# zhide1983/audio_codec

Measured on AMD Instinct MI355X. Metric: Mframes/s encoded (48kHz/10ms/64kbps), higher is better.
Workload: dtype f32

## Files before the change

audio_codec_amd/csrc/lc3_enc_front4.inc:

```
#define F4_FR 4
#define F4_N 480
#define F4_CS 36
#define F4_ZS 544
struct __attribute__((aligned(16))) Front4Lds {
    float x[MEMCAP + F4_FR * F4_N + 4];
    float scr[364];
    int   pc[LC3D_PLAN_HEAD_WORDS];
    int   cc[14];
};
static_assert(MEMCAP % 4 == 0 && F4_FR * F4_ZS <= MEMCAP + F4_FR * F4_N, "front4 work buffers fit into the PCM area");

__device__ __forceinline__ void f4_dft240x4(float* x, const lc3d_plan* __restrict__ P, float norm, int lane)
{
    constexpr int N = F4_N;
    {
        const int f = lane >> 4, col = lane & 15;
        if (col < 15) {
            float* z = &x[F4_ZS * f + F4_CS * col];
            float v[32];
#pragma unroll
            for (int q = 0; q < 8; q++) { const float4 u = *(const float4*)&z[4 * q]; v[4 * q] = u.x; v[4 * q + 1] = u.y; v[4 * q + 2] = u.z; v[4 * q + 3] = u.w; }
            dft16(v);
#pragma unroll
            for (int q = 0; q < 8; q++) *(float4*)&z[4 * q] = make_float4(v[4 * q], v[4 * q + 1], v[4 * q + 2], v[4 * q + 3]);
        }
    }
    LSYNC();
    {
        const int f = lane >> 4, row = lane & 15;
        float v[30];
#pragma unroll
        for (int l = 0; l < 15; l++) { const float2 u = *(const float2*)&x[F4_ZS * f + F4_CS * l + 2 * row]; v[2 * l] = u.x; v[2 * l + 1] = u.y; }
        dft15(v);
        float o0[15], o1[15];
#pragma unroll
        for (int l = 0; l < 15; l++) {
            const unsigned tt = 15u * row + 16u * l, d = tt < tt - 240u ? tt : tt - 240u;
            const float2 tw = *(const float2*)&P->tw2[2 * d];
            const float ar = v[2 * l], ai = v[2 * l + 1];
            const float tr = ar * tw.x - ai * tw.y, ti = ai * tw.x + ar * tw.y;
            o0[l] = tr * norm; o1[l] = -ti * norm;
        }
        LSYNC();
        float* A = &x[N * f];
#pragma unroll
        for (int l = 0; l < 15; l++) {
            const unsigned tt = 15u * row + 16u * l, d = tt < tt - 240u ? tt : tt - 240u;
            A[2 * d] = o0[l]; A[N - 2 * d - 1] = o1[l];
        }
    }
    LSYNC();
}

#ifndef F4_WAVES
#define F4_WAVES 4
#endif
extern "C" __global__ void __launch_bounds__(WAVE) __attribute__((amdgpu_waves_per_eu(F4_WAVES, F4_WAVES)))
#ifdef LC3_PCM_FMT
lc3_enc_front4_kernel_fmt(
#else
lc3_enc_front4_kernel(
#endif
                      const lc3d_plan* __restrict__ P, const lc3d_chan* __restrict__ chans, const float* __restrict__ state, const void* __restrict__ pcm, int bitdepth,
                      int T, int tb, int nt , int ncs, float* __restrict__ spec, int srow, int RT, int r0, float* __restrict__ rec,
                      float* __restrict__ xnext, const float* __restrict__ xprev, int xprev_stride)
{
    __shared__ Front4Lds L;
    const int lane = threadIdx.x;
    const int runs = (nt + F4_FR - 1) / F4_FR;
    const int cs = blockIdx.x / runs, t0 = tb + (blockIdx.x % runs) * F4_FR, nf = imin(F4_FR, tb + nt - t0);
    if (cs >= ncs) return;
    if (lane < LC3D_PLAN_HEAD_WORDS) L.pc[lane] = ((const int*)P)[lane];
    if (lane < 14) L.cc[lane] = ((const int*)&chans[cs])[lane];
    LSYNC();
    constexpr int N = F4_N, h = N / 2;
    const int channels = PI(channels);
    const int strm = cs / channels, ch = cs - strm * channels;
#ifndef LC3_PCM_FMT
    const float sc = bitdepth == 24 ? 256.0f : 65536.0f;
#endif
#ifdef LC3_PCM_FMT
    {
        const int ps = lc3d_pcm_stride(bitdepth, channels);
        const size_t pf0 = lc3d_pcm_frame(bitdepth, channels, T, N, strm, t0, ch), pfst = lc3d_pcm_fstep(bitdepth, channels, N);
        const bool fastf = pcm_f32_wide(pcm, bitdepth, pf0, N) && ((pfst * 4) & 15) == 0;
        if (t0 == 0) { for (int i = lane; i < MEMCAP; i += WAVE) L.x[i] = xprev[(size_t)cs * xprev_stride + i]; }
        else {
            const size_t pidx = pf0 - pfst + (size_t)(N - MEMCAP) * ps;
            if (fastf) {
                const float4* p = (const float4*)((const float*)pcm + pidx);
                for (int j = lane; j < MEMCAP / 4; j += WAVE) *(float4*)&L.x[4 * j] = pcm_f32x4(p[j]);
            } else for (int j = lane; j < MEMCAP; j += WAVE) L.x[j] = pcm_in(pcm, bitdepth, pidx + (size_t)j * ps);
        }
        if (fastf) {
            for (int idx = lane; idx < 120 * nf; idx += WAVE) {
                const int f = idx / 120, j = idx - 120 * f;
                *(float4*)&L.x[MEMCAP + N * f + 4 * j] = pcm_f32x4(((const float4*)((const float*)pcm + pf0 + (size_t)f * pfst))[j]);
            }
        } else {
            for (int f = 0; f < nf; f++) {
                const size_t o = pf0 + (size_t)f * pfst;
                for (int i = lane; i < N; i += WAVE) L.x[MEMCAP + N * f + i] = pcm_in(pcm, bitdepth, o + (size_t)i * ps);
            }
        }
    }
#else
    {
        const size_t f0 = ((size_t)strm * T + t0) * channels + ch;
        const bool fast = bitdepth == 16 && (((size_t)pcm) & 15) == 0;
        if (t0 == 0) { for (int i = lane; i < MEMCAP; i += WAVE) L.x[i] = xprev[(size_t)cs * xprev_stride + i]; }
        else {
            const size_t pidx = (f0 - channels) * N + (N - MEMCAP);
            if (fast) {
                const uint2* p = (const uint2*)((const int16_t*)pcm + pidx);
                for (int j = lane; j < MEMCAP / 4; j += WAVE) {
                    const uint2 v = p[j];
                    *(float4*)&L.x[4 * j] = make_float4((float)(int16_t)(v.x & 0xffff), (float)(int16_t)(v.x >> 16), (float)(int16_t)(v.y & 0xffff), (float)(int16_t)(v.y >> 16));
                }
            } else for (int j = lane; j < MEMCAP; j += WAVE)
                L.x[j] = bitdepth == 16 ? (float)((const int16_t*)pcm)[pidx + j] : (float)((const int32_t*)pcm)[pidx + j] / sc;
        }
        if (fast) {
#pragma unroll
            for (int k = 0; k < 4; k++) {
                const int idx = lane + 64 * k, f = idx / 60, j = idx - 60 * f;
                if (idx < 240 && f < nf) {
#ifdef F4_NOLOAD
                    const uint4 v = make_uint4(idx * 77u, idx * 131u, idx * 17u, idx * 3u);
#else
                    const uint4 v = ((const uint4*)((const int16_t*)pcm + (f0 + (size_t)f * channels) * N))[j];
#endif
                    float* d = &L.x[MEMCAP + N * f + 8 * j];
                    *(float4*)&d[0] = make_float4((float)(int16_t)(v.x & 0xffff), (float)(int16_t)(v.x >> 16), (float)(int16_t)(v.y & 0xffff), (float)(int16_t)(v.y >> 16));
                    *(float4*)&d[4] = make_float4((float)(int16_t)(v.z & 0xffff), (float)(int16_t)(v.z >> 16), (float)(int16_t)(v.w & 0xffff), (float)(int16_t)(v.w >> 16));
                }
            }
        } else {
            for (int f = 0; f < nf; f++) {
                const size_t o = (f0 + (size_t)f * channels) * N;
                for (int i = lane; i < N; i += WAVE)
                    L.x[MEMCAP + N * f + i] = bitdepth == 16 ? (float)((const int16_t*)pcm)[o + i] : (float)((const int32_t*)pcm)[o + i] / sc;
            }
        }
    }
#endif
    LSYNC();
    if (t0 + nf == T) for (int i = lane; i < MEMCAP; i += WAVE) xnext[(size_t)cs * MEMCAP + i] = L.x[N * nf + i];
    float* r = rec + ((size_t)cs * RT + r0 + t0) * FR_WORDS;
    if (lane < nf) ((int*)r)[(size_t)lane * FR_WORDS + FR_ATTFLAG] = 0;
    if (CI(attack_handling) != 0) {
        const float* stp = state + (size_t)cs * LC3D_STATE_WORDS(MEMCAP);
        float am0 = 0, am1 = 0;
        for (int f = 0; f < nf; f++) {
            if (t0 + f == 0) { if (!CI(reset_attack)) { am0 = stp[LC3D_ST_SCAL(MEMCAP) + F_ATT_M0]; am1 = stp[LC3D_ST_SCAL(MEMCAP) + F_ATT_M1]; } }
            else if (f == 0) { const float* q = &L.x[MEMCAP]; am0 = (q[-6] + q[-5] + q[-4]); am1 = (q[-3] + q[-2] + q[-1]); }
            float n0, n1;
            const float e = attack_energies_at(PI(att_nblocks), 48000, &L.x[MEMCAP + N * f], L.scr, lane, am0, am1, n0, n1);
            float* rf = r + (size_t)f * FR_WORDS;
            if (lane < 4) rf[FR_ATT + lane] = lane < PI(att_nblocks) ? e : 0.0f;
            if (lane == 0) { rf[FR_ATTM] = n0; rf[FR_ATTM + 1] = n1; }
            am0 = n0; am1 = n1;
            LSYNC();
        }
    }
    const float* w = &lc3t_win_pool[PI(win_off)];
    const int lim = 2 * N - PI(la);
    float zr[4][F4_FR], zi[4][F4_FR];
    if (lane < 60) {
#pragma unroll
        for (int k = 0; k < 4; k++) {
            const int i = lane + 60 * k;
            const int m1 = k < 2 ? 2 * i : N - 1 - 2 * i, m2 = k < 2 ? h - 1 - 2 * i : 2 * i - h;
            const int j0 = 3 * h - m1 - 1, j1 = 3 * h + m1, j2 = m2, j3 = 2 * h - m2 - 1;
            const float w0 = w[j0], w1 = w[j1], w2 = w[j2], w3 = w[j3];
            const float2 tw = *(const float2*)&P->tw1[2 * i];
            const bool in1 = j1 < lim; const int j1c = in1 ? j1 : 0;
#pragma unroll
            for (int f = 0; f < F4_FR; f++) {
                const float* t = &L.x[N * f];
                const float a0 = t[j0] * w0;
                const float a1 = (in1 ? t[j1c] : 0.0f) * w1;
                const float a2 = t[j2] * w2;
                const float a3 = t[j3] * w3;
                const float F1 = -a0 - a1, F2 = a2 - a3;
                const float ar = k < 2 ? F1 : F2, ai = k < 2 ? F2 : F1;
                zr[k][f] = ar * tw.x - ai * tw.y;
                zi[k][f] = ai * tw.x + ar * tw.y;
            }
        }
    }
    LSYNC();
    if (lane < 60) {
#pragma unroll
        for (int k = 0; k < 4; k++) {
            const int i = lane + 60 * k;
            const int o = (i % 15) * F4_CS + 2 * (i & 15);
#pragma unroll
            for (int f = 0; f < F4_FR; f++) *(float2*)&L.x[F4_ZS * f + o] = make_float2(zr[k][f], zi[k][f]);
        }
    }
    LSYNC();
    f4_dft240x4(L.x, P, PF(dct4_norm), lane);
    {
        const int nq = PI(ylen);
        float* base = LC3D_ROW_BASE(spec, cs, r0 + t0, RT, srow);
        for (int idx = lane; idx < nq; idx += WAVE) {
            const int c = idx >> 4, f = (idx >> 2) & 3, q = idx & 3;
            if (f < nf) *(float4*)&base[((size_t)c * RT + f) * 16 + 4 * q] = *(const float4*)&L.x[N * f + 16 * c + 4 * q];
        }
    }
}
```

audio_codec_amd/csrc/lc3_enc_shapel.inc:

```
#ifndef LC3_BIG
struct __attribute__((aligned(16))) ShlLds {
    double l10[128 * 3];
    double ex2[64];
    unsigned bob[LC3D_MAX_N / 4];
    int   pc[LC3D_PLAN_HEAD_WORDS];
};

__device__ __attribute__((noinline)) void shl_lpc_weight(const float* a_in, const float* rc_in, float* outp, int maxOrder, float maxPG, float predGain)
{
    float sc[36], pa[9];
    pa[0] = 1;
    for (int j = 1; j <= maxOrder - 1; j++) pa[j] = -a_in[maxOrder - j];
    pa[maxOrder] = rc_in[maxOrder - 1];
    const float alpha = (float)((double)((maxPG - predGain)) * (0.85f - 1.0) / (double)(maxPG - 1.5f) + 1.0);
    for (int i = 0; i <= maxOrder; i++) sc[i] = pa[i] * m_powf(alpha, (float)i);
    int len = maxOrder + 1; const int len0 = len;
    float* pa_ = sc; float* out = sc + 9; float* t0 = sc + 18; float* bf = sc + 26;
    for (int i = 0; i < len - 1; i++) out[i] = 0;
    { float a0 = pa_[0]; for (int i = 0; i < len; i++) { pa_[i] = pa_[i] / a0; a0 = pa_[0]; } }
    out[len - 1] = pa_[len - 1];
    for (int k = len0 - 2; k >= 0; k--) {
        for (int i = 0; i < len - 1; i++) t0[i] = pa_[1 + i];
        int l = len - 1;
        const float knxt = t0[l - 1];
// ... 18 lines not shown
#define SHL_ATTR __attribute__((amdgpu_waves_per_eu(SHL_WAVES, SHL_WAVES), amdgpu_num_vgpr(SHL_VGPRS)))
#else
#define SHL_ATTR __attribute__((amdgpu_waves_per_eu(SHL_WAVES, SHL_WAVES)))
#endif
#ifdef LC3_ENC_VBW
#define SHL_KERNEL_NAME lc3_enc_shape_lane_kernel_vbw
#else
#define SHL_KERNEL_NAME lc3_enc_shape_lane_kernel
#endif
extern "C" __global__ void __launch_bounds__(WAVE) SHL_ATTR
SHL_KERNEL_NAME(const lc3d_plan* __restrict__ P, const lc3d_chan* __restrict__ chans, int RT , int r0 , int nt, int ncs,
                          float* __restrict__ rows , int srow, float* __restrict__ frec
#ifdef LC3_ENC_VBW
                          , const uint16_t* __restrict__ bwf
#endif
                          )
{
    __shared__ ShlLds L;
    const int lane = threadIdx.x;
    if (lane < LC3D_PLAN_HEAD_WORDS) L.pc[lane] = ((const int*)P)[lane];
    for (int i = lane; i < LC3D_MAX_N; i += WAVE) ((uint8_t*)L.bob)[i] = P->band_of_bin[i];
    for (int i = lane; i < 128 * 3; i += WAVE) L.l10[i] = lc3m_log10_tab[i];
    L.ex2[lane] = lc3m_exp2_tab[lane];
    LSYNC();
#if !defined(LC3_OCML_MATH) && !defined(SHL_GLOBAL_TABLES)
#define m_log10f(x_) lc3m_log10f((x_), L.l10)
#define m_pow2f(x_) lc3m_exp2f((x_), L.ex2)
#endif
    const long long cf = (long long)blockIdx.x * WAVE + lane;
    const bool valid = cf < (long long)ncs * nt;
    const int cs = valid ? (int)(cf / nt) : 0, t = valid ? r0 + (int)(cf % nt) : r0;
    float* xr = LC3D_ROW_BASE(rows, cs, t, RT, srow);
#define XP(k_) (&xr[LC3D_ROW_OFF((k_), RT)])
    float* rec = frec + ((size_t)cs * RT + t) * FR_WORDS;
    const lc3d_chan* __restrict__ C = &chans[cs];
    const int ylen = PI(ylen), N = PI(N), nb = PI(nbands), dms = PI(dms), hr = PI(hrmode);
    const int total_bits = C->total_bits, off = C->gg_off;
    float g[16];
#pragma unroll
    for (int i = 0; i < 16; i += 4) { const float4 v = *(const float4*)&rec[FR_SCFQ + i]; g[i] = v.x; g[i + 1] = v.y; g[i + 2] = v.z; g[i + 3] = v.w; }
    const int dnb = 64 - nb;
    int n4 = 0;
    if (dnb >= 32) { const float ratio = fabsf((float)(1.0 - 32.0 / (double)(float)nb)); n4 = (int)round((double)(ratio * (float)nb)); }
    auto v64 = [&](int i) -> float {
        float ga, gb; int r;
        if (i < 2) return g[0];
        if (i < 62) { const int n = (i - 2) >> 2; r = (i - 2) & 3; ga = g[n]; gb = g[n + 1]; }
        else { ga = g[15]; gb = g[15]; r = i - 62; const double dd = (double)(g[15] - g[14]); return r == 0 ? (float)((double)ga + dd / 8.0) : (float)((double)ga + 3.0 * dd / 8.0); }
        const double dd = (double)(gb - ga);
        if (r == 0) return (float)((double)ga + dd / 8.0);
        if (r == 1) return (float)((double)ga + 3.0 * dd / 8.0);
        if (r == 2) return (float)((double)ga + 5.0 * dd / 8.0);
        return (float)((double)ga + 7.0 * dd / 8.0);
    };
    auto band_gain = [&](int b) -> float {
        float v;
        if (dnb == 0) v = v64(b);
        else if (dnb < 32) { if (b < dnb) v = (float)((double)(v64(2 * b) + v64(2 * b + 1)) / 2.0); else v = v64(b + dnb); }
        else {
            if (b < n4) v = (float)((double)(v64(4 * b) + v64(4 * b + 1) + v64(4 * b + 2) + v64(4 * b + 3)) / 4.0);
            else { const int i = b - n4; v = (float)((double)(v64(4 * n4 + 2 * i) + v64(4 * n4 + 2 * i + 1)) / 2.0); }
        }
        return m_pow2f(-v);
    };
    int bw = ((const int*)rec)[FR_BW];
#ifdef LC3_ENC_VBW
// ... 5 lines not shown
    if (cut) bw = imin(bw, C->bw_index);
#endif
    const int bw_bin = lc3t_bw_bins[PI(bw_cls) * 6 + bw];
    int numfilters, start0, start1 = 0, stop0, stop1 = 0, obits_off = 8; float maxPG = 2;
    const int maxOrder = dms == 100 ? 8 : 4, nSub = dms == 100 ? 3 : 2;
    {
        int fs = PI(fs), Nn = N;
        numfilters = (fs >= 32000 && dms >= 50) ? 2 : 1;
        if ((double)Nn > 40 * ((double)(float)dms / 10.0)) { Nn = (int)(40 * ((double)(float)dms / 10.0)); fs = 40000; }
        start0 = (600 * Nn * 2 / fs) + 1;
        if ((dms >= 50 && (double)total_bits >= 48 * ((double)(float)dms / 10.0)) || dms == 25) { maxPG = 1.5f; obits_off = 0; }
        if (bw >= 3 && numfilters == 2) { start1 = bw_bin / 2 + 1; stop0 = bw_bin / 2; stop1 = bw_bin; }
        else { numfilters = 1; stop0 = bw_bin; }
    }
    float R0[9], R1[9];
#pragma unroll
    for (int k = 0; k < 9; k++) { R0[k] = 0; R1[k] = 0; }
    {
        float acc[9], rr[9], yp[8];
#pragma unroll
        for (int k = 0; k < 9; k++) { acc[k] = 0; rr[k] = 0; }
#pragma unroll
        for (int k = 0; k < 8; k++) yp[k] = 0;
        int cur_b = -1; float cur_g = 1.0f;
        int sf = 0, ssub = 0; bool dead = false;
        int slo, shi;
#define SHL_BOUNDS() do { const int fstart_ = sf ? start1 : start0, fstop_ = sf ? stop1 : stop0; \
            const float sublen_ = (float)(((double)(float)fstop_ + 1.0 - (double)(float)fstart_) / (double)(float)nSub); \
            slo = (int)(floor((double)(sublen_ * (float)ssub)) + fstart_ - 1); shi = (int)(floor((double)(sublen_ * (float)(ssub + 1))) + fstart_ - 1); \
            if (sf >= numfilters) { slo = 0x7fffffff; shi = 0x7fffffff; } } while (0)
        SHL_BOUNDS();
        float4 xn[4];
#pragma unroll
        for (int j = 0; j < 4; j++) xn[j] = *(const float4*)XP(4 * j);
        for (int k0 = 0; k0 < ylen; k0 += 16) {
            float xs[16], ys[16];
#pragma unroll
            for (int j = 0; j < 4; j++) { xs[4 * j] = xn[j].x; xs[4 * j + 1] = xn[j].y; xs[4 * j + 2] = xn[j].z; xs[4 * j + 3] = xn[j].w; }
            if (k0 + 16 < ylen) {
#pragma unroll
                for (int j = 0; j < 4; j++) xn[j] = *(const float4*)XP(k0 + 16 + 4 * j);
            }
            const unsigned bw4[4] = {L.bob[(k0 >> 2)], L.bob[(k0 >> 2) + 1], L.bob[(k0 >> 2) + 2], L.bob[(k0 >> 2) + 3]};
#pragma unroll
            for (int j = 0; j < 16; j++) {
                const int b = uni((int)((bw4[j >> 2] >> (8 * (j & 3))) & 255u)), k = k0 + j;
                if (b != cur_b) { cur_b = b; cur_g = b < nb ? band_gain(b) : 1.0f; }
                float y = k < ylen ? xs[j] : 0.0f;
                if (b < nb) y = y * cur_g;
                ys[j] = y;
            }
            if (__any(cut && ylen > cbin && k0 + 16 > cbin - 1)) {
#pragma unroll
                for (int j = 0; j < 16; j++) {
                    const int k = k0 + j;
                    if (cut && ylen > cbin) {
                        if (k >= cbin - 1 && k < cbin + 3) ys[j] = ys[j] * (k == cbin - 1 ? 0.5f : k == cbin ? 0.25f : k == cbin + 1 ? 0.125f : 0.0625f);
                        else if (k >= cbin + 3) ys[j] = 0;
                    }
                }
            }
#ifndef SHL_RESHAPE_B
            if (valid) {
#pragma unroll
                for (int j = 0; j < 4; j++) if (k0 + 4 * j < ylen) *(float4*)XP(k0 + 4 * j) = make_float4(ys[4 * j], ys[4 * j + 1], ys[4 * j + 2], ys[4 * j + 3]);
            }
#endif
            if (__all(k0 - slo >= 8 && k0 + 16 <= shi)) {
#pragma unroll
                for (int j = 0; j < 16; j++) {
#pragma unroll
                    for (int k = 0; k < 9; k++) { const float h = j - k >= 0 ? ys[j - k >= 0 ? j - k : 0] : yp[8 + j - k >= 0 ? 8 + j - k : 0]; acc[k] += ys[j] * h; }
                }
            } else if (__any(k0 + 16 > slo && k0 <= shi)) {
// ... 106 lines not shown
                int ix = 0;
#pragma unroll
                for (int q = 0; q < 17; q++) ix = (c <= lc3t_tns_rc_thr[q + 1] && c > lc3t_tns_rc_thr[q]) ? q : ix;
                if (i >= maxOrder) ix = 0;
                idx[i] = ix;
                qv[i] = (tns && i < maxOrder) ? lc3t_tns_rc_pts[ix] : 0.0f;
                if (qv[i] != 0) o = i + 1;
            }
            if (o == 0) tns = 0;
            int bits = live ? 1 : 0;
            if (tns) {
                int tsum = 0;
#pragma unroll
                for (int i = 0; i < 8; i++) if (i < o) tsum += lc3t_tns_coef_bits[i * 17 + idx[i]];
                bits += (tsum + lc3t_tns_order_bits[obits_off + o - 1] + 2047) >> 11;
            }
            tns_bits += bits;
            ord[f] = tns ? o : 0;
#pragma unroll
            for (int i = 0; i < 8; i++) { rcq[f][i] = live ? qv[i] : 0.0f; tidx[f][i] = (tns && i < o) ? idx[i] : 0; }
        }
    }
    const bool anyf = ord[0] > 0 || ord[1] > 0;
    const bool regul = hr && C->reg_bits > 0;
    float x_max = 0; float M0 = 1e-5f, M1 = 1e-5f;
    {
        float st[8], rca[8]; bool tm[8];
#pragma unroll
        for (int j = 0; j < 8; j++) { st[j] = 0; rca[j] = rcq[0][j]; tm[j] = j < ord[0]; }
        int phase = 0, nextev = numfilters == 2 ? start1 - 1 : stop0;
        int cur_b = -1; float cur_g = 1.0f;
        float4 xn[4];
#pragma unroll
        for (int j = 0; j < 4; j++) xn[j] = *(const float4*)XP(4 * j);
        for (int k0 = 0; k0 < ylen; k0 += 16) {
            float ys[16];
#pragma unroll
            for (int j = 0; j < 4; j++) { ys[4 * j] = xn[j].x; ys[4 * j + 1] = xn[j].y; ys[4 * j + 2] = xn[j].z; ys[4 * j + 3] = xn[j].w; }
            if (k0 + 16 < ylen) {
#pragma unroll
                for (int j = 0; j < 4; j++) xn[j] = *(const float4*)XP(k0 + 16 + 4 * j);
            }
#ifdef SHL_RESHAPE_B
            {
                const unsigned bw4[4] = {L.bob[(k0 >> 2)], L.bob[(k0 >> 2) + 1], L.bob[(k0 >> 2) + 2], L.bob[(k0 >> 2) + 3]};
#pragma unroll
                for (int j = 0; j < 16; j++) {
                    const int b = uni((int)((bw4[j >> 2] >> (8 * (j & 3))) & 255u)), k = k0 + j;
                    if (b != cur_b) { cur_b = b; cur_g = b < nb ? band_gain(b) : 1.0f; }
                    float y = k < ylen ? ys[j] : 0.0f;
                    if (b < nb) y = y * cur_g;
                    ys[j] = y;
                }
                if (__any(cut && ylen > cbin && k0 + 16 > cbin - 1)) {
#pragma unroll
                    for (int j = 0; j < 16; j++) {
                        const int k = k0 + j;
                        if (cut && ylen > cbin) {
                            if (k >= cbin - 1 && k < cbin + 3) ys[j] = ys[j] * (k == cbin - 1 ? 0.5f : k == cbin ? 0.25f : k == cbin + 1 ? 0.125f : 0.0625f);
                            else if (k >= cbin + 3) ys[j] = 0;
                        }
                    }
                }
            }
#endif
#ifdef SHL_RESHAPE_B
            const bool changed = true;
#else
            const bool changed = __any(anyf && k0 + 16 > start0 - 1 && k0 < (numfilters == 2 ? stop1 : stop0));
#endif
            if (__any(anyf && k0 + 16 > start0 - 1 && k0 < (numfilters == 2 ? stop1 : stop0))) {
                const int comax = uni(wave_max_i(imax(ord[0], ord[1])));
#pragma unroll
                for (int j = 0; j < 16; j++) {
// ... 78 lines not shown
        const float thresh = 2 * PF(frame_ms);
        const float q = M1 / M0;
        const float rB = 8 * (1 - (q < thresh ? q : thresh) / thresh);
        const float reg_val = regul ? x_max * m_powf(2.0f, (float)(-C->reg_bits) - rB) : 0.0f;
        for (int k0 = 0; k0 < ylen; k0 += 16) {
            float ys[16], e4[4];
#pragma unroll
            for (int j = 0; j < 4; j++) { const float4 v = *(const float4*)XP(k0 + 4 * j); ys[4 * j] = v.x; ys[4 * j + 1] = v.y; ys[4 * j + 2] = v.z; ys[4 * j + 3] = v.w; }
#pragma unroll
            for (int q2 = 0; q2 < 4; q2++) {
                float tt = ys[4 * q2] * ys[4 * q2];
                tt += ys[4 * q2 + 1] * ys[4 * q2 + 1]; tt += ys[4 * q2 + 2] * ys[4 * q2 + 2]; tt += ys[4 * q2 + 3] * ys[4 * q2 + 3];
                e4[q2] = (float)((28.0 / 20.0) * (7 + 10.0 * (double)m_log10f(tt + reg_val + PF(c_2m31))));
            }
            if (valid && regul) *(float4*)XP(ylen + (k0 >> 2)) = make_float4(e4[0], e4[1], e4[2], e4[3]);
        }
    }
    float ind_min = (float)off;
    if (x_max != 0) {
        const float g_min = hr == 1 ? x_max / (float)(32768 * 256 - 2) : (float)((double)x_max / (32768 - 0.375));
        ind_min = (float)ceil(28.0 * (double)m_log10f(g_min));
    }
    if (valid) {
        int* ri = (int*)rec;
        *(int4*)&ri[FR_TNS] = make_int4(numfilters, ord[0], ord[1], tns_bits);
#pragma unroll
        for (int f = 0; f < 2; f++) {
            *(int4*)&ri[FR_TNS + 4 + 8 * f] = make_int4(tidx[f][0], tidx[f][1], tidx[f][2], tidx[f][3]);
            *(int4*)&ri[FR_TNS + 8 + 8 * f] = make_int4(tidx[f][4], tidx[f][5], tidx[f][6], tidx[f][7]);
        }
        ri[FR_GGMIN] = __float_as_int(ind_min); ri[FR_XZERO] = x_max == 0 ? 1 : 0; ri[FR_BWC] = bw;
    }
#undef XP
#undef m_log10f
#undef m_pow2f
}
#endif

#if !defined(LC3_BIG) && !defined(LC3_ENC_VBW)
struct __attribute__((aligned(16))) ScfLds {
    float en[64 * 64];
    int   be[68];
    int   pc[LC3D_PLAN_HEAD_WORDS];
};
#ifndef SCF_WAVES
#define SCF_WAVES 3
#endif
extern "C" __global__ void __launch_bounds__(WAVE) __attribute__((amdgpu_waves_per_eu(SCF_WAVES, SCF_WAVES)))
lc3_enc_scf_lane_kernel(const lc3d_plan* __restrict__ P, int RT, int r0, int nt, int ncs, const float* __restrict__ rows , int srow, float* __restrict__ frec,
                        int with_vq )
{
    __shared__ ScfLds L;
    const int lane = threadIdx.x;
    if (lane < LC3D_PLAN_HEAD_WORDS) L.pc[lane] = ((const int*)P)[lane];
    LSYNC();
    const int nb0 = PI(nbands), ylen = PI(ylen);
    for (int i = lane; i < 68; i += WAVE) L.be[i] = i <= nb0 ? (int)lc3t_band_pool[PI(band_off) + i] : 0x7fffffff;
    LSYNC();
    const long long cf = (long long)blockIdx.x * WAVE + lane;
    const bool valid = cf < (long long)ncs * nt;
    const int cs = valid ? (int)(cf / nt) : 0, t = valid ? r0 + (int)(cf % nt) : r0;
    const float* xr = LC3D_ROW_BASE(rows, cs, t, RT, srow);
#define XP(k_) (&xr[LC3D_ROW_OFF((k_), RT)])
    float* rec = frec + ((size_t)cs * RT + t) * FR_WORDS;
    {
        int b = 0, edge = uni(L.be[1]), lo = uni(L.be[0]);
        float sum = 0;
        float4 xn[4];
#pragma unroll
        for (int j = 0; j < 4; j++) xn[j] = *(const float4*)XP(4 * j);
        for (int k0 = 0; k0 < ylen; k0 += 16) {
            float xs[16];
#pragma unroll
            for (int j = 0; j < 4; j++) { xs[4 * j] = xn[j].x; xs[4 * j + 1] = xn[j].y; xs[4 * j + 2] = xn[j].z; xs[4 * j + 3] = xn[j].w; }
            if (k0 + 16 < ylen) {
#pragma unroll
                for (int j = 0; j < 4; j++) xn[j] = *(const float4*)XP(k0 + 16 + 4 * j);
            }
#pragma unroll
            for (int j = 0; j < 16; j++) {
                const int k = k0 + j;
                while (k == edge) {
                    L.en[b * 64 + lane] = sum / (float)(edge - lo);
                    sum = 0; b++; lo = edge; edge = uni(L.be[b + 1]);
                }
                if (k < ylen) sum += xs[j] * xs[j];
            }
        }
        while (b < nb0) { L.en[b * 64 + lane] = sum / (float)(edge - lo); sum = 0; b++; lo = edge; edge = uni(L.be[b + 1]); }
    }
    int bw = PI(fs_idx);
    if (PI(fs_idx) > 0 && PI(hrmode) == 0) {
        const int f = PI(fs_idx);
        const uint8_t* st = &lc3t_bw_start[(PI(bw_cls) * 4 + f - 1) * 4]; const uint8_t* sp = &lc3t_bw_stop[(PI(bw_cls) * 4 + f - 1) * 4];
        int counter = f;
        float sum = 0;
        for (int i = st[counter - 1]; i <= sp[counter - 1]; i++) sum += L.en[i * 64 + lane];
        float mean = sum / (float)(sp[counter - 1] - st[counter - 1] + 1);
        while (mean < (float)lc3t_bw_quiet_thr[counter - 1]) {
            counter--;
            if (counter == 0) break;
            sum = 0;
            for (int i = st[counter - 1]; i <= sp[counter - 1]; i++) sum += L.en[i * 64 + lane];
            mean = sum / (float)(sp[counter - 1] - st[counter - 1] + 1);
        }
        bw = counter;
        if (bw < f) {
            const float thr = (float)lc3t_bw_brick_thr[counter];
            const int stop = st[counter], dist = lc3t_bw_brick_dist[counter];
            int brick = 0;
            for (int i = stop; i >= stop - dist; i--) {
                const float ediff = (float)(10.0 * (double)m_log10f(L.en[(i - dist + 1) * 64 + lane] + 1.1920928955078125e-07f) -
                                            10.0 * (double)m_log10f(L.en[(i + 1) * 64 + lane] + 1.1920928955078125e-07f));
                if (ediff > thr) { brick = 1; break; }
            }
            if (!brick) bw = f;
        }
    }
    const int d = 64 - nb0;
// ... 72 lines not shown
```

audio_codec_amd/csrc/lc3_launch.h:

```cpp
#ifndef LC3_LAUNCH_H
#define LC3_LAUNCH_H
#include "lc3_plan.h"

#define WAVE 64
#define IMDCT_FPW 8
#ifndef FRONT_FPW
#define FRONT_FPW 4
#endif
#ifndef FM_F240
#define FM_F240 4
#endif
#ifndef PRE_FPW
#define PRE_FPW 8
#endif
#define PRE96_ITERS 4
#ifndef SHAPE_FPW
#define SHAPE_FPW 4
#endif
#define RATE_WG 4
#define PK_XBUF 16
#define PKS_THREADS 256
#define PKS_ITEMS 8
#define PKS_TILE (PKS_THREADS * PKS_ITEMS)
struct PkSrc { const uint16_t* fsz; const int4* pend; const lc3d_chan* chans; int channels, order, S, T; };
struct __attribute__((aligned(16))) ParseLds {
    unsigned short cum[64 * 32 + 8];
    unsigned short tcum[18 + 144];
    unsigned char lut[4096];
    unsigned mpvq[176];
    int pc[LC3D_PLAN_HEAD_WORDS];
};
#endif
```

audio_codec_amd/csrc/lc3_runtime.hip:

```cpp
#include <hip/hip_runtime.h>
#include <stdint.h>
#include <stdio.h>
#include <stdlib.h>
#include <string.h>

#include "lc3_plan.h"
#include "lc3_shim.h"
#include "lc3_launch.h"
#include "lc3_kernel_decls.h"

#define LC3D_MAX_RUNS 16
#ifndef LC3D_SETS
#define LC3D_SETS 3
#endif
#define LC3D_AHEAD_MAX_FRAMES 256
#define LC3D_RUN_FRAMES 16
#define LC3D_RUN_FRAMES_READY 64
struct lc3hip_opts {
    int fused, no_split, streams5, run_frames, runs, ahead_max, rate_stream , pre_runs, pitch2, scf_wave, front4, shape_fpw, shape_on_s, shape_wave,
        pack_wpg, pack_stream , resample48, resample96, dec_imdct4, check_ready, tailw_bytes, dec_parse_pad_kb, pack_pad_kb, pack_split, pack_w5, fuse_vq, stream_order, stream_skip, rate_on, dec_plc_stream, shape_on_pitch, side_prio;
};
static int env_int(const char* name, int lo, int hi, int dflt) { const char* e = getenv(name); if (!e || !*e) return dflt; const int v = atoi(e); return v >= lo && v <= hi ? v : dflt; }
static void read_opts(lc3hip_opts* o)
{
// ... 354 lines not shown
            HIPCHK(hipEventRecord(c->ev_fork, s)); HIPCHK(hipStreamWaitEvent(c->s_pre, c->ev_fork, 0)); HIPCHK(hipStreamWaitEvent(c->s_fr, c->ev_fork, 0));
            if (five) { HIPCHK(hipStreamWaitEvent(c->s_pit, c->ev_fork, 0)); HIPCHK(hipStreamWaitEvent(c->s_ln, c->ev_fork, 0)); }
        } else {
            HIPCHK(hipStreamWaitEvent(c->s_pre, c->ev_m[R - 1], 0));
            HIPCHK(hipStreamWaitEvent(c->s_pre, c->ev_done[hb_], 0)); HIPCHK(hipStreamWaitEvent(c->s_fr, c->ev_done[hb_], 0));
            if (five) { HIPCHK(hipStreamWaitEvent(c->s_pit, c->ev_done[hb_], 0)); HIPCHK(hipStreamWaitEvent(c->s_ln, c->ev_done[hb_], 0));
                        if (c->any_attack) HIPCHK(hipStreamWaitEvent(c->s_fr, c->ev_f[R - 1], 0)); }
        }
        hipStream_t rs = s;
        for (int k = 0, tb = 0, hb = 0, hk = 0; tb < n_frames; k++, tb += Tr) {
            const int nt = n_frames - tb < Tr ? n_frames - tb : Tr;
            if (tb >= hb) {
                const int prn = c->opt.pre_runs;
                const int hn0 = hk == 0 ? Tr : prn * Tr, hn = n_frames - hb < hn0 ? n_frames - hb : hn0;
                DUPL('r') launch_resample(c, c->s_pre, dpcm, bitdepth, n_frames, hb, hn, mc, dy12, xprev, xprev_stride);
                DUPL('h') hipLaunchKernelGGL(lc3_enc_hp50_kernel, dim3((unsigned)((c->ncs + WAVE - 1) / WAVE)), dim3(WAVE), 0, c->s_pre, c->d_plan, c->d_state, c->state_words, LC3D_ST_SCAL(mc), n_frames, hb, hn, c->ncs, dy12);
                HIPCHK(hipGetLastError());
                hb += hn; hk++;
                if (five) { HIPCHK(hipEventRecord(c->ev_h[k], c->s_pre)); HIPCHK(hipStreamWaitEvent(c->s_pit, c->ev_h[k], 0)); }
            }
            const int p2 = c->opt.pitch2;
            if (p2 && (c->len12 == 128 || c->len12 == 64 || c->len12 == 32)) {
                auto pk = c->len12 == 128 ? lc3_enc_pitch2_kernel : c->len12 == 64 ? lc3_enc_pitch2_kernel_l64 : lc3_enc_pitch2_kernel_l32;
                DUPL('p') hipLaunchKernelGGL(pk, dim3((unsigned)((c->ncs + 1) / 2)), dim3(WAVE), 0, c->s_pit, c->d_plan, c->d_chans, c->d_state, c->state_words, mc, dy12, n_frames, tb, nt, c->ncs, dfrec, dT, dt0);
            }
            else DUPL('p') hipLaunchKernelGGL(lc3_enc_pitch_kernel, dim3(c->ncs), dim3(WAVE), 0, c->s_pit, c->d_plan, c->d_chans, c->d_state, c->state_words, mc, dy12, n_frames, tb, nt, c->ncs, dfrec, dT, dt0);
            HIPCHK(hipGetLastError());
            HIPCHK(hipEventRecord(c->ev_p[k], c->s_pit));
            const int scf_wave = c->opt.scf_wave;
            const int fpw = nt < FRONT_FPW ? nt : FRONT_FPW;
            const unsigned fruns = (unsigned)((nt + fpw - 1) / fpw);
            const int f4 = c->opt.front4;
            if (f4 && !c->big && !scf_wave && c->N == 480 && c->la == 180 && (c->ylen & 15) == 0)
                DUPL('f') hipLaunchKernelGGL(fmt_plain ? lc3_enc_front4_kernel : lc3_enc_front4_kernel_fmt, dim3((unsigned)c->ncs * (unsigned)((nt + 3) / 4)), dim3(WAVE), 0, c->s_fr, c->d_plan, c->d_chans, c->d_state, dpcm, bitdepth, n_frames, tb, nt, c->ncs, dspec, c->srow, dT, dt0, dfrec, xn_w, xprev, xprev_stride);
            else if (f4 && c->fm_frames && !scf_wave)
                hipLaunchKernelGGL(fmt_plain ? lc3_enc_frontm_kernel : lc3_enc_frontm_kernel_fmt, dim3((unsigned)c->ncs * (unsigned)((nt + c->fm_frames - 1) / c->fm_frames)), dim3(WAVE), 0, c->s_fr, c->d_plan, c->d_chans, c->d_state, dpcm, bitdepth, n_frames, tb, nt, c->fm_frames, c->ncs, dspec, c->srow, dT, dt0, dfrec, xn_w, xprev, xprev_stride);
            else if (c->big) hipLaunchKernelGGL(fmt_plain ? lc3_enc_front_kernel_big : lc3_enc_front_kernel_big_fmt, dim3((unsigned)c->ncs * fruns), dim3(WAVE), 0, c->s_fr, c->d_plan, c->d_chans, c->d_state, dpcm, bitdepth, n_frames, tb, nt, fpw, c->ncs, dspec, c->srow, dT, dt0, dfrec, xn_w, xprev, xprev_stride, scf_wave);
            else DUPL('f') hipLaunchKernelGGL(fmt_plain ? lc3_enc_front_kernel : lc3_enc_front_kernel_fmt, dim3((unsigned)c->ncs * fruns), dim3(WAVE), 0, c->s_fr, c->d_plan, c->d_chans, c->d_state, dpcm, bitdepth, n_frames, tb, nt, fpw, c->ncs, dspec, c->srow, dT, dt0, dfrec, xn_w, xprev, xprev_stride, scf_wave);
            HIPCHK(hipEventRecord(c->ev_m[k], c->s_fr));
            if (five) HIPCHK(hipStreamWaitEvent(c->s_ln, c->ev_m[k], 0));
            const int fuse_vq = !scf_wave && !c->any_attack && c->opt.fuse_vq;
            if (!scf_wave) DUPL('e') hipLaunchKernelGGL(lc3_enc_scf_lane_kernel, dim3((unsigned)(((long long)c->ncs * nt + WAVE - 1) / WAVE)), dim3(WAVE), 0, c->s_ln, c->d_plan, dT, dt0 + tb, nt, c->ncs, dspec, c->srow, dfrec, fuse_vq);
            if (c->any_attack)
                hipLaunchKernelGGL(lc3_enc_attack_kernel, dim3((unsigned)((c->ncs + WAVE - 1) / WAVE)), dim3(WAVE), 0, c->s_ln, c->d_plan, c->d_chans, c->d_state, c->state_words, LC3D_ST_SCAL(mc), dfrec, dT, dt0, tb, nt, c->ncs);
            const long long nfr = (long long)c->ncs * nt;
            if (!fuse_vq) DUPL('v') hipLaunchKernelGGL(lc3_enc_snsvq_kernel, dim3((unsigned)((nfr + WAVE - 1) / WAVE)), dim3(WAVE), 0, c->s_ln, c->d_plan, dfrec, dT, dt0, tb, nt, c->ncs, c->any_attack);
            {
                const int sfpw = c->opt.shape_fpw ? c->opt.shape_fpw : SHAPE_FPW, son = c->opt.shape_on_s;
                const int spw = nt < sfpw ? nt : sfpw;
                const unsigned sruns = (unsigned)((nt + spw - 1) / spw);
                const bool sop = !son && (c->opt.shape_on_pitch >= 0 ? c->opt.shape_on_pitch == 1 : (c->hr && c->N == 240 && n_frames >= 128));
                hipStream_t ss = son ? s : sop ? c->s_pit : c->s_ln;
                rs = (son || !rts) ? s : rts;
                if (son) { HIPCHK(hipEventRecord(c->ev_f[k], c->s_ln)); HIPCHK(hipStreamWaitEvent(s, c->ev_f[k], 0)); }
                if (sop) { HIPCHK(hipEventRecord(c->ev_v[k], c->s_ln)); HIPCHK(hipStreamWaitEvent(ss, c->ev_v[k], 0)); }
                const int swave = c->opt.shape_wave;
                if (dbw && bw_to(c, ss)) return 1;
                if (dbw && !swave) hipLaunchKernelGGL(lc3_enc_shape_lane_kernel_vbw, dim3((unsigned)(((long long)c->ncs * nt + WAVE - 1) / WAVE)), dim3(WAVE), 0, ss, c->d_plan, c->d_chans, dT, dt0 + tb, nt, c->ncs, dspec, c->srow, dfrec, dbw);
                else if (dbw) hipLaunchKernelGGL(lc3_enc_shape_kernel_vbw, dim3((unsigned)c->ncs * sruns), dim3(WAVE), 0, ss, c->d_plan, c->d_chans, dT, dt0 + tb, nt, spw, c->ncs, dspec, c->srow, dfrec, dbw);
                else if (!swave) DUPL('a') hipLaunchKernelGGL(lc3_enc_shape_lane_kernel, dim3((unsigned)(((long long)c->ncs * nt + WAVE - 1) / WAVE)), dim3(WAVE), 0, ss, c->d_plan, c->d_chans, dT, dt0 + tb, nt, c->ncs, dspec, c->srow, dfrec);
                else if (c->big) hipLaunchKernelGGL(lc3_enc_shape_kernel_big, dim3((unsigned)c->ncs * sruns), dim3(WAVE), 0, ss, c->d_plan, c->d_chans, dT, dt0 + tb, nt, spw, c->ncs, dspec, c->srow, dfrec);
                else DUPL('a') hipLaunchKernelGGL(lc3_enc_shape_kernel, dim3((unsigned)c->ncs * sruns), dim3(WAVE), 0, ss, c->d_plan, c->d_chans, dT, dt0 + tb, nt, spw, c->ncs, dspec, c->srow, dfrec);
                HIPCHK(hipGetLastError());
                if (!son) { HIPCHK(hipEventRecord(c->ev_f[k], ss)); HIPCHK(hipStreamWaitEvent(rs, c->ev_f[k], 0)); }
            }
            HIPCHK(hipStreamWaitEvent(rs, c->ev_p[k], 0));
            if (k == 0 && c->rate_armed) HIPCHK(hipStreamWaitEvent(rs, c->ev_rate, 0));
// ... 854 lines not shown
```

Before: 116.0.

## Let front4 workgroups walk multiple runs with PCM prefetch; deepen scf load lookahead

The front4 kernel can now process several consecutive 4-frame runs per workgroup (F4_WALK). It carries the MDCT overlap memory through LDS instead of reloading it from PCM, and issues the next run's PCM loads early so they overlap the DFT. Window and twiddle loads are hoisted to the start of each iteration. The scf lane kernel keeps SCF_AHEAD blocks of row loads in flight instead of one, to hide memory latency at the cost of extra registers. With F4_WALK defaulting to 1, the walk path stays inactive and only the load reordering and deeper scf prefetch take effect.

```diff
diff --git a/audio_codec_amd/csrc/lc3_enc_front4.inc b/audio_codec_amd/csrc/lc3_enc_front4.inc
--- a/audio_codec_amd/csrc/lc3_enc_front4.inc
+++ b/audio_codec_amd/csrc/lc3_enc_front4.inc
@@ -8,7 +8,7 @@
     int   pc[LC3D_PLAN_HEAD_WORDS];
     int   cc[14];
 };
-static_assert(MEMCAP % 4 == 0 && F4_FR * F4_ZS <= MEMCAP + F4_FR * F4_N, "front4 work buffers fit into the PCM area");
+static_assert(MEMCAP % 4 == 0 && MEMCAP <= 364 && F4_FR * F4_ZS <= MEMCAP + F4_FR * F4_N, "front4 work buffers fit into the PCM area");
 
 __device__ __forceinline__ void f4_dft240x4(float* x, const lc3d_plan* __restrict__ P, float norm, int lane)
 {
@@ -55,6 +55,9 @@
 #ifndef F4_WAVES
 #define F4_WAVES 4
 #endif
+#ifndef F4_PCM_EARLY
+#define F4_PCM_EARLY 2
+#endif
 extern "C" __global__ void __launch_bounds__(WAVE) __attribute__((amdgpu_waves_per_eu(F4_WAVES, F4_WAVES)))
 #ifdef LC3_PCM_FMT
 lc3_enc_front4_kernel_fmt(
@@ -67,8 +70,8 @@
 {
     __shared__ Front4Lds L;
     const int lane = threadIdx.x;
-    const int runs = (nt + F4_FR - 1) / F4_FR;
-    const int cs = blockIdx.x / runs, t0 = tb + (blockIdx.x % runs) * F4_FR, nf = imin(F4_FR, tb + nt - t0);
+    const int runs = (nt + F4_FR - 1) / F4_FR, wgs = (runs + F4_WALK - 1) / F4_WALK;
+    const int cs = blockIdx.x / wgs, run0 = (blockIdx.x % wgs) * F4_WALK, nw = imin(F4_WALK, runs - run0);
     if (cs >= ncs) return;
     if (lane < LC3D_PLAN_HEAD_WORDS) L.pc[lane] = ((const int*)P)[lane];
     if (lane < 14) L.cc[lane] = ((const int*)&chans[cs])[lane];
@@ -78,76 +81,119 @@
     const int strm = cs / channels, ch = cs - strm * channels;
 #ifndef LC3_PCM_FMT
     const float sc = bitdepth == 24 ? 256.0f : 65536.0f;
-#endif
-#ifdef LC3_PCM_FMT
-    {
-        const int ps = lc3d_pcm_stride(bitdepth, channels);
-        const size_t pf0 = lc3d_pcm_frame(bitdepth, channels, T, N, strm, t0, ch), pfst = lc3d_pcm_fstep(bitdepth, channels, N);
-        const bool fastf = pcm_f32_wide(pcm, bitdepth, pf0, N) && ((pfst * 4) & 15) == 0;
-        if (t0 == 0) { for (int i = lane; i < MEMCAP; i += WAVE) L.x[i] = xprev[(size_t)cs * xprev_stride + i]; }
+    const bool fast = bitdepth == 16 && (((size_t)pcm) & 15) == 0;
+    auto pcm_request = [&](uint4 (&pq)[4], int ka, int kb, int ln_, int t0_, int nf_) {
+        const size_t f0_ = ((size_t)strm * T + t0_) * channels + ch;
+#pragma unroll
+        for (int k = 0; k < 4; k++) {
+            if (k < ka || k >= kb) continue;
+            const int idx = ln_ + 64 * k, f = idx / 60, j = idx - 60 * f, fc = imin(f, nf_ - 1);
+#ifdef F4_NOLOAD
+            pq[k] = make_uint4(idx * 77u, idx * 131u, idx * 17u, idx * 3u);
+#else
+            pq[k] = ((const uint4*)((const int16_t*)pcm + (f0_ + (size_t)fc * channels) * N))[j];
+#endif
+        }
+    };
+    auto pcm_to_x = [&](const uint4 (&pq)[4], int ln_, int nf_) {
+#pragma unroll
+        for (int k = 0; k < 4; k++) {
+            const int idx = ln_ + 64 * k, f = idx / 60, j = idx - 60 * f;
+            if (idx < 240 && f < nf_) {
+                const uint4 v = pq[k];
+                float* d = &L.x[MEMCAP + N * f + 8 * j];
+                *(float4*)&d[0] = make_float4((float)(int16_t)(v.x & 0xffff), (float)(int16_t)(v.x >> 16), (float)(int16_t)(v.y & 0xffff), (float)(int16_t)(v.y >> 16));
+                *(float4*)&d[4] = make_float4((float)(int16_t)(v.z & 0xffff), (float)(int16_t)(v.z >> 16), (float)(int16_t)(v.w & 0xffff), (float)(int16_t)(v.w >> 16));
+            }
+        }
+    };
+#endif
+#pragma unroll 1
+    for (int wk = 0; wk < nw; wk++) {
+    int ln = lane, zo = 0;
+    asm volatile("" : "+v"(ln), "+s"(zo));
+    ln &= WAVE - 1;
+#ifdef LC3_PCM_FMT
+    const void* pcw = (const char*)pcm + zo; int bdw = bitdepth;
+    asm volatile("" : "+s"(bdw));
+#endif
+    const float* w = &lc3t_win_pool[PI(win_off)];
+    const int lim = 2 * N - PI(la);
+    float wv[4][4]; float2 twv[4];
+    auto win_request = [&](int ln_, const lc3d_plan* P_) {
+#pragma unroll
+        for (int k = 0; k < 4; k++) {
+            const int i = imin(ln_, 59) + 60 * k;
+            const int m1 = k < 2 ? 2 * i : N - 1 - 2 * i, m2 = k < 2 ? h - 1 - 2 * i : 2 * i - h;
+            wv[k][0] = w[3 * h - m1 - 1]; wv[k][1] = w[3 * h + m1]; wv[k][2] = w[m2]; wv[k][3] = w[2 * h - m2 - 1];
+            twv[k] = *(const float2*)&P_->tw1[2 * i];
+        }
+    };
+    const int t0 = tb + (run0 + wk) * F4_FR, nf = imin(F4_FR, tb + nt - t0);
+#ifndef LC3_PCM_FMT
+    win_request(ln, P);
+#endif
+#ifdef LC3_PCM_FMT
+    {
+        const int ps = lc3d_pcm_stride(bdw, channels);
+        const size_t pf0 = lc3d_pcm_frame(bdw, channels, T, N, strm, t0, ch), pfst = lc3d_pcm_fstep(bdw, channels, N);
+        const bool fastf = pcm_f32_wide(pcw, bdw, pf0, N) && ((pfst * 4) & 15) == 0;
+        if (wk > 0) {
+            for (int i = ln; i < MEMCAP; i += WAVE) L.x[i] = L.scr[i];
+        }
+        else if (t0 == 0) { for (int i = ln; i < MEMCAP; i += WAVE) L.x[i] = xprev[(size_t)cs * xprev_stride + i]; }
         else {
             const size_t pidx = pf0 - pfst + (size_t)(N - MEMCAP) * ps;
             if (fastf) {
-                const float4* p = (const float4*)((const float*)pcm + pidx);
-                for (int j = lane; j < MEMCAP / 4; j += WAVE) *(float4*)&L.x[4 * j] = pcm_f32x4(p[j]);
-            } else for (int j = lane; j < MEMCAP; j += WAVE) L.x[j] = pcm_in(pcm, bitdepth, pidx + (size_t)j * ps);
+                const float4* p = (const float4*)((const float*)pcw + pidx);
+                for (int j = ln; j < MEMCAP / 4; j += WAVE) *(float4*)&L.x[4 * j] = pcm_f32x4(p[j]);
+            } else for (int j = ln; j < MEMCAP; j += WAVE) L.x[j] = pcm_in(pcw, bdw, pidx + (size_t)j * ps);
         }
         if (fastf) {
-            for (int idx = lane; idx < 120 * nf; idx += WAVE) {
+            for (int idx = ln; idx < 120 * nf; idx += WAVE) {
                 const int f = idx / 120, j = idx - 120 * f;
-                *(float4*)&L.x[MEMCAP + N * f + 4 * j] = pcm_f32x4(((const float4*)((const float*)pcm + pf0 + (size_t)f * pfst))[j]);
+                *(float4*)&L.x[MEMCAP + N * f + 4 * j] = pcm_f32x4(((const float4*)((const float*)pcw + pf0 + (size_t)f * pfst))[j]);
             }
         } else {
             for (int f = 0; f < nf; f++) {
                 const size_t o = pf0 + (size_t)f * pfst;
-                for (int i = lane; i < N; i += WAVE) L.x[MEMCAP + N * f + i] = pcm_in(pcm, bitdepth, o + (size_t)i * ps);
+                for (int i = ln; i < N; i += WAVE) L.x[MEMCAP + N * f + i] = pcm_in(pcw, bdw, o + (size_t)i * ps);
             }
         }
     }
 #else
     {
         const size_t f0 = ((size_t)strm * T + t0) * channels + ch;
-        const bool fast = bitdepth == 16 && (((size_t)pcm) & 15) == 0;
-        if (t0 == 0) { for (int i = lane; i < MEMCAP; i += WAVE) L.x[i] = xprev[(size_t)cs * xprev_stride + i]; }
+        if (wk > 0) {
+            for (int i = ln; i < MEMCAP; i += WAVE) L.x[i] = L.scr[i];
+        }
+        else if (t0 == 0) { for (int i = ln; i < MEMCAP; i += WAVE) L.x[i] = xprev[(size_t)cs * xprev_stride + i]; }
         else {
             const size_t pidx = (f0 - channels) * N + (N - MEMCAP);
             if (fast) {
                 const uint2* p = (const uint2*)((const int16_t*)pcm + pidx);
-                for (int j = lane; j < MEMCAP / 4; j += WAVE) {
+                for (int j = ln; j < MEMCAP / 4; j += WAVE) {
                     const uint2 v = p[j];
                     *(float4*)&L.x[4 * j] = make_float4((float)(int16_t)(v.x & 0xffff), (float)(int16_t)(v.x >> 16), (float)(int16_t)(v.y & 0xffff), (float)(int16_t)(v.y >> 16));
                 }
-            } else for (int j = lane; j < MEMCAP; j += WAVE)
+            } else for (int j = ln; j < MEMCAP; j += WAVE)
                 L.x[j] = bitdepth == 16 ? (float)((const int16_t*)pcm)[pidx + j] : (float)((const int32_t*)pcm)[pidx + j] / sc;
         }
         if (fast) {
-#pragma unroll
-            for (int k = 0; k < 4; k++) {
-                const int idx = lane + 64 * k, f = idx / 60, j = idx - 60 * f;
-                if (idx < 240 && f < nf) {
-#ifdef F4_NOLOAD
-                    const uint4 v = make_uint4(idx * 77u, idx * 131u, idx * 17u, idx * 3u);
-#else
-                    const uint4 v = ((const uint4*)((const int16_t*)pcm + (f0 + (size_t)f * channels) * N))[j];
-#endif
-                    float* d = &L.x[MEMCAP + N * f + 8 * j];
-                    *(float4*)&d[0] = make_float4((float)(int16_t)(v.x & 0xffff), (float)(int16_t)(v.x >> 16), (float)(int16_t)(v.y & 0xffff), (float)(int16_t)(v.y >> 16));
-                    *(float4*)&d[4] = make_float4((float)(int16_t)(v.z & 0xffff), (float)(int16_t)(v.z >> 16), (float)(int16_t)(v.w & 0xffff), (float)(int16_t)(v.w >> 16));
-                }
-            }
+            if (wk == 0) { uint4 pq[4]; pcm_request(pq, 0, 4, ln, t0, nf); pcm_to_x(pq, ln, nf); }
         } else {
             for (int f = 0; f < nf; f++) {
                 const size_t o = (f0 + (size_t)f * channels) * N;
-                for (int i = lane; i < N; i += WAVE)
+                for (int i = ln; i < N; i += WAVE)
                     L.x[MEMCAP + N * f + i] = bitdepth == 16 ? (float)((const int16_t*)pcm)[o + i] : (float)((const int32_t*)pcm)[o + i] / sc;
             }
         }
     }
 #endif
     LSYNC();
-    if (t0 + nf == T) for (int i = lane; i < MEMCAP; i += WAVE) xnext[(size_t)cs * MEMCAP + i] = L.x[N * nf + i];
+    if (t0 + nf == T) for (int i = ln; i < MEMCAP; i += WAVE) xnext[(size_t)cs * MEMCAP + i] = L.x[N * nf + i];
     float* r = rec + ((size_t)cs * RT + r0 + t0) * FR_WORDS;
-    if (lane < nf) ((int*)r)[(size_t)lane * FR_WORDS + FR_ATTFLAG] = 0;
+    if (ln < nf) ((int*)r)[(size_t)ln * FR_WORDS + FR_ATTFLAG] = 0;
     if (CI(attack_handling) != 0) {
         const float* stp = state + (size_t)cs * LC3D_STATE_WORDS(MEMCAP);
         float am0 = 0, am1 = 0;
@@ -155,25 +201,26 @@
             if (t0 + f == 0) { if (!CI(reset_attack)) { am0 = stp[LC3D_ST_SCAL(MEMCAP) + F_ATT_M0]; am1 = stp[LC3D_ST_SCAL(MEMCAP) + F_ATT_M1]; } }
             else if (f == 0) { const float* q = &L.x[MEMCAP]; am0 = (q[-6] + q[-5] + q[-4]); am1 = (q[-3] + q[-2] + q[-1]); }
             float n0, n1;
-            const float e = attack_energies_at(PI(att_nblocks), 48000, &L.x[MEMCAP + N * f], L.scr, lane, am0, am1, n0, n1);
+            const float e = attack_energies_at(PI(att_nblocks), 48000, &L.x[MEMCAP + N * f], L.scr, ln, am0, am1, n0, n1);
             float* rf = r + (size_t)f * FR_WORDS;
-            if (lane < 4) rf[FR_ATT + lane] = lane < PI(att_nblocks) ? e : 0.0f;
-            if (lane == 0) { rf[FR_ATTM] = n0; rf[FR_ATTM + 1] = n1; }
+            if (ln < 4) rf[FR_ATT + ln] = ln < PI(att_nblocks) ? e : 0.0f;
+            if (ln == 0) { rf[FR_ATTM] = n0; rf[FR_ATTM + 1] = n1; }
             am0 = n0; am1 = n1;
             LSYNC();
         }
     }
-    const float* w = &lc3t_win_pool[PI(win_off)];
-    const int lim = 2 * N - PI(la);
+#ifdef LC3_PCM_FMT
+    win_request(ln, P);
+#endif
     float zr[4][F4_FR], zi[4][F4_FR];
-    if (lane < 60) {
-#pragma unroll
-        for (int k = 0; k < 4; k++) {
-            const int i = lane + 60 * k;
+    if (ln < 60) {
+#pragma unroll
+        for (int k = 0; k < 4; k++) {
+            const int i = ln + 60 * k;
             const int m1 = k < 2 ? 2 * i : N - 1 - 2 * i, m2 = k < 2 ? h - 1 - 2 * i : 2 * i - h;
             const int j0 = 3 * h - m1 - 1, j1 = 3 * h + m1, j2 = m2, j3 = 2 * h - m2 - 1;
-            const float w0 = w[j0], w1 = w[j1], w2 = w[j2], w3 = w[j3];
-            const float2 tw = *(const float2*)&P->tw1[2 * i];
+            const float w0 = wv[k][0], w1 = wv[k][1], w2 = wv[k][2], w3 = wv[k][3];
+            const float2 tw = twv[k];
             const bool in1 = j1 < lim; const int j1c = in1 ? j1 : 0;
 #pragma unroll
             for (int f = 0; f < F4_FR; f++) {
@@ -190,23 +237,39 @@
         }
     }
     LSYNC();
-    if (lane < 60) {
-#pragma unroll
-        for (int k = 0; k < 4; k++) {
-            const int i = lane + 60 * k;
+    if (wk + 1 < nw) { for (int i = ln; i < MEMCAP; i += WAVE) L.scr[i] = L.x[N * F4_FR + i]; LSYNC(); }
+#ifndef LC3_PCM_FMT
+    const bool ahead = fast && wk + 1 < nw;
+    uint4 pq[4] = {};
+    if (ahead) pcm_request(pq, 0, F4_PCM_EARLY, ln, t0 + F4_FR, imin(F4_FR, tb + nt - t0 - F4_FR));
+#endif
+    if (ln < 60) {
+#pragma unroll
+        for (int k = 0; k < 4; k++) {
+            const int i = ln + 60 * k;
             const int o = (i % 15) * F4_CS + 2 * (i & 15);
 #pragma unroll
             for (int f = 0; f < F4_FR; f++) *(float2*)&L.x[F4_ZS * f + o] = make_float2(zr[k][f], zi[k][f]);
         }
     }
     LSYNC();
-    f4_dft240x4(L.x, P, PF(dct4_norm), lane);
+    f4_dft240x4(L.x, P, PF(dct4_norm), ln);
+#ifndef LC3_PCM_FMT
+    if (ahead) pcm_request(pq, F4_PCM_EARLY, 4, ln, t0 + F4_FR, imin(F4_FR, tb + nt - t0 - F4_FR));
+#endif
     {
         const int nq = PI(ylen);
         float* base = LC3D_ROW_BASE(spec, cs, r0 + t0, RT, srow);
-        for (int idx = lane; idx < nq; idx += WAVE) {
+        for (int idx = ln; idx < nq; idx += WAVE) {
             const int c = idx >> 4, f = (idx >> 2) & 3, q = idx & 3;
             if (f < nf) *(float4*)&base[((size_t)c * RT + f) * 16 + 4 * q] = *(const float4*)&L.x[N * f + 16 * c + 4 * q];
         }
     }
+    if (wk + 1 < nw) {
+        LSYNC();
+#ifndef LC3_PCM_FMT
+        if (ahead) pcm_to_x(pq, ln, imin(F4_FR, tb + nt - t0 - F4_FR));
+#endif
+    }
+    }
 }
diff --git a/audio_codec_amd/csrc/lc3_enc_shapel.inc b/audio_codec_amd/csrc/lc3_enc_shapel.inc
--- a/audio_codec_amd/csrc/lc3_enc_shapel.inc
+++ b/audio_codec_amd/csrc/lc3_enc_shapel.inc
@@ -74,6 +74,11 @@
     const int cs = valid ? (int)(cf / nt) : 0, t = valid ? r0 + (int)(cf % nt) : r0;
     float* xr = LC3D_ROW_BASE(rows, cs, t, RT, srow);
 #define XP(k_) (&xr[LC3D_ROW_OFF((k_), RT)])
+#ifdef SHL_NOLOAD
+#define SHL_ROW4(k_) make_float4((float)((lane * 77 + (k_) * 131) & 1023) - 512.0f, (float)((lane * 17 + (k_) * 3) & 1023) - 511.0f, (float)((lane * 5 + (k_) * 29) & 511) - 256.0f, (float)((lane + (k_) * 7) & 255) - 127.0f)
+#else
+#define SHL_ROW4(k_) (*(const float4*)XP(k_))
+#endif
     float* rec = frec + ((size_t)cs * RT + t) * FR_WORDS;
     const lc3d_chan* __restrict__ C = &chans[cs];
     const int ylen = PI(ylen), N = PI(N), nb = PI(nbands), dms = PI(dms), hr = PI(hrmode);
@@ -145,14 +150,14 @@
         SHL_BOUNDS();
         float4 xn[4];
 #pragma unroll
-        for (int j = 0; j < 4; j++) xn[j] = *(const float4*)XP(4 * j);
+        for (int j = 0; j < 4; j++) xn[j] = SHL_ROW4(4 * j);
         for (int k0 = 0; k0 < ylen; k0 += 16) {
             float xs[16], ys[16];
 #pragma unroll
             for (int j = 0; j < 4; j++) { xs[4 * j] = xn[j].x; xs[4 * j + 1] = xn[j].y; xs[4 * j + 2] = xn[j].z; xs[4 * j + 3] = xn[j].w; }
             if (k0 + 16 < ylen) {
 #pragma unroll
-                for (int j = 0; j < 4; j++) xn[j] = *(const float4*)XP(k0 + 16 + 4 * j);
+                for (int j = 0; j < 4; j++) xn[j] = SHL_ROW4(k0 + 16 + 4 * j);
             }
             const unsigned bw4[4] = {L.bob[(k0 >> 2)], L.bob[(k0 >> 2) + 1], L.bob[(k0 >> 2) + 2], L.bob[(k0 >> 2) + 3]};
 #pragma unroll
@@ -325,14 +330,14 @@
         int cur_b = -1; float cur_g = 1.0f;
         float4 xn[4];
 #pragma unroll
-        for (int j = 0; j < 4; j++) xn[j] = *(const float4*)XP(4 * j);
+        for (int j = 0; j < 4; j++) xn[j] = SHL_ROW4(4 * j);
         for (int k0 = 0; k0 < ylen; k0 += 16) {
             float ys[16];
 #pragma unroll
             for (int j = 0; j < 4; j++) { ys[4 * j] = xn[j].x; ys[4 * j + 1] = xn[j].y; ys[4 * j + 2] = xn[j].z; ys[4 * j + 3] = xn[j].w; }
             if (k0 + 16 < ylen) {
 #pragma unroll
-                for (int j = 0; j < 4; j++) xn[j] = *(const float4*)XP(k0 + 16 + 4 * j);
+                for (int j = 0; j < 4; j++) xn[j] = SHL_ROW4(k0 + 16 + 4 * j);
             }
 #ifdef SHL_RESHAPE_B
             {
@@ -477,6 +482,7 @@
         ri[FR_GGMIN] = __float_as_int(ind_min); ri[FR_XZERO] = x_max == 0 ? 1 : 0; ri[FR_BWC] = bw;
     }
 #undef XP
+#undef SHL_ROW4
 #undef m_log10f
 #undef m_pow2f
 }
@@ -490,6 +496,9 @@
 };
 #ifndef SCF_WAVES
 #define SCF_WAVES 3
+#endif
+#ifndef SCF_AHEAD
+#define SCF_AHEAD 4
 #endif
 extern "C" __global__ void __launch_bounds__(WAVE) __attribute__((amdgpu_waves_per_eu(SCF_WAVES, SCF_WAVES)))
 lc3_enc_scf_lane_kernel(const lc3d_plan* __restrict__ P, int RT, int r0, int nt, int ncs, const float* __restrict__ rows , int srow, float* __restrict__ frec,
@@ -511,25 +520,34 @@
     {
         int b = 0, edge = uni(L.be[1]), lo = uni(L.be[0]);
         float sum = 0;
-        float4 xn[4];
-#pragma unroll
-        for (int j = 0; j < 4; j++) xn[j] = *(const float4*)XP(4 * j);
-        for (int k0 = 0; k0 < ylen; k0 += 16) {
-            float xs[16];
-#pragma unroll
-            for (int j = 0; j < 4; j++) { xs[4 * j] = xn[j].x; xs[4 * j + 1] = xn[j].y; xs[4 * j + 2] = xn[j].z; xs[4 * j + 3] = xn[j].w; }
-            if (k0 + 16 < ylen) {
-#pragma unroll
-                for (int j = 0; j < 4; j++) xn[j] = *(const float4*)XP(k0 + 16 + 4 * j);
-            }
-#pragma unroll
-            for (int j = 0; j < 16; j++) {
-                const int k = k0 + j;
-                while (k == edge) {
-                    L.en[b * 64 + lane] = sum / (float)(edge - lo);
-                    sum = 0; b++; lo = edge; edge = uni(L.be[b + 1]);
-                }
-                if (k < ylen) sum += xs[j] * xs[j];
+        const int klast = (ylen - 1) & ~15;
+        float4 xn[SCF_AHEAD][4];
+#pragma unroll
+        for (int s = 0; s < SCF_AHEAD; s++) {
+            const int kq = imin(16 * s, klast);
+#pragma unroll
+            for (int j = 0; j < 4; j++) xn[s][j] = *(const float4*)XP(kq + 4 * j);
+        }
+        for (int kb = 0; kb < ylen; kb += 16 * SCF_AHEAD) {
+#pragma unroll
+            for (int s = 0; s < SCF_AHEAD; s++) {
+                const int k0 = kb + 16 * s;
+                if (k0 >= ylen) break;
+                float xs[16];
+#pragma unroll
+                for (int j = 0; j < 4; j++) { xs[4 * j] = xn[s][j].x; xs[4 * j + 1] = xn[s][j].y; xs[4 * j + 2] = xn[s][j].z; xs[4 * j + 3] = xn[s][j].w; }
+                const int kq = imin(k0 + 16 * SCF_AHEAD, klast);
+#pragma unroll
+                for (int j = 0; j < 4; j++) xn[s][j] = *(const float4*)XP(kq + 4 * j);
+#pragma unroll
+                for (int j = 0; j < 16; j++) {
+                    const int k = k0 + j;
+                    while (k == edge) {
+                        L.en[b * 64 + lane] = sum / (float)(edge - lo);
+                        sum = 0; b++; lo = edge; edge = uni(L.be[b + 1]);
+                    }
+                    if (k < ylen) sum += xs[j] * xs[j];
+                }
             }
         }
         while (b < nb0) { L.en[b * 64 + lane] = sum / (float)(edge - lo); sum = 0; b++; lo = edge; edge = uni(L.be[b + 1]); }
diff --git a/audio_codec_amd/csrc/lc3_launch.h b/audio_codec_amd/csrc/lc3_launch.h
--- a/audio_codec_amd/csrc/lc3_launch.h
+++ b/audio_codec_amd/csrc/lc3_launch.h
@@ -6,6 +6,9 @@
 #define IMDCT_FPW 8
 #ifndef FRONT_FPW
 #define FRONT_FPW 4
+#endif
+#ifndef F4_WALK
+#define F4_WALK 1
 #endif
 #ifndef FM_F240
 #define FM_F240 4
diff --git a/audio_codec_amd/csrc/lc3_runtime.hip b/audio_codec_amd/csrc/lc3_runtime.hip
--- a/audio_codec_amd/csrc/lc3_runtime.hip
+++ b/audio_codec_amd/csrc/lc3_runtime.hip
@@ -410,7 +410,7 @@
             const unsigned fruns = (unsigned)((nt + fpw - 1) / fpw);
             const int f4 = c->opt.front4;
             if (f4 && !c->big && !scf_wave && c->N == 480 && c->la == 180 && (c->ylen & 15) == 0)
-                DUPL('f') hipLaunchKernelGGL(fmt_plain ? lc3_enc_front4_kernel : lc3_enc_front4_kernel_fmt, dim3((unsigned)c->ncs * (unsigned)((nt + 3) / 4)), dim3(WAVE), 0, c->s_fr, c->d_plan, c->d_chans, c->d_state, dpcm, bitdepth, n_frames, tb, nt, c->ncs, dspec, c->srow, dT, dt0, dfrec, xn_w, xprev, xprev_stride);
+                DUPL('f') hipLaunchKernelGGL(fmt_plain ? lc3_enc_front4_kernel : lc3_enc_front4_kernel_fmt, dim3((unsigned)c->ncs * (unsigned)(((nt + 3) / 4 + F4_WALK - 1) / F4_WALK)), dim3(WAVE), 0, c->s_fr, c->d_plan, c->d_chans, c->d_state, dpcm, bitdepth, n_frames, tb, nt, c->ncs, dspec, c->srow, dT, dt0, dfrec, xn_w, xprev, xprev_stride);
             else if (f4 && c->fm_frames && !scf_wave)
                 hipLaunchKernelGGL(fmt_plain ? lc3_enc_frontm_kernel : lc3_enc_frontm_kernel_fmt, dim3((unsigned)c->ncs * (unsigned)((nt + c->fm_frames - 1) / c->fm_frames)), dim3(WAVE), 0, c->s_fr, c->d_plan, c->d_chans, c->d_state, dpcm, bitdepth, n_frames, tb, nt, c->fm_frames, c->ncs, dspec, c->srow, dT, dt0, dfrec, xn_w, xprev, xprev_stride);
             else if (c->big) hipLaunchKernelGGL(fmt_plain ? lc3_enc_front_kernel_big : lc3_enc_front_kernel_big_fmt, dim3((unsigned)c->ncs * fruns), dim3(WAVE), 0, c->s_fr, c->d_plan, c->d_chans, c->d_state, dpcm, bitdepth, n_frames, tb, nt, fpw, c->ncs, dspec, c->srow, dT, dt0, dfrec, xn_w, xprev, xprev_stride, scf_wave);
```

Measured after the change: 102.4. -11.7%, worse.
